# sharonct/CTPA-CLIP

Measured on AMD Instinct MI355X. Metric: CT-report pairs/sec (contrastive step), higher is better.
Workload: dtype bf16

## Files before the change

ctpa-clip_amd/csrc/attn.hip:

```cpp
#include "common.h"
#include "../../include/ctclip_hip.h"

namespace {

constexpr float LOG2E = 1.4426950408889634f;
constexpr float LN2 = 0.6931471805599453f;

struct AP {
  const u16* q; int64_t ldq;
  const u16* k; int64_t ldk;
  const u16* v; int64_t ldv;
  const u16* o; int64_t ldo;
  u16* out; int64_t ldout;
  u16* out16;
  const u16* dout; int64_t lddo;
  u16* dq; int64_t lddq;
  u16* dk; int64_t lddk;
  u16* dv; int64_t lddv;
  float* lse;
  float* delta;
  const float* bias_u;
  float* dbias_u;
  float* dbias_ws;
  const int32_t* kmask;
// ... 655 lines not shown
        pk.y = pack2(dq[d][2], dq[d][3]);
        *(uint2*)(p.dq + qrow * p.lddq + h * D + d * 16 + 4 * g) = pk;
      }
    }
  }
  if (BIAS && p.dbias_u) {
    __syncthreads();
    const int hh = blockIdx.x % p.H;
    for (int i = tid; i < p.nbins; i += NT) {
      const float v = bins[i];
      if (v != 0.f) atomicAdd(&p.dbias_u[(int64_t)hh * p.nbins + i], v);
    }
  }
}

template <int D, bool BIAS, int W = (BIAS ? 12 : NW), bool RUN = false>
__global__ __launch_bounds__(W * 64) void attn_bwd_dkv_kernel(AP p) {
  extern __shared__ __attribute__((aligned(16))) char smem[];
  constexpr int KK = D / 32, DB = D / 16, RS = Img<D>::RS, NTH = W * 64;
  const int L = p.L, Lp = (L + 31) & ~31;
  const int tid = threadIdx.x, lane = tid & 63, w = tid >> 6;
  const int wpp = W / p.pp;
  const int pair_local = w / wpp, wi = w - pair_local * wpp;
  const int pair_bytes = 2 * Lp * RS + 2 * Lp * 4;
  for (int pl = 0; pl < p.pp; ++pl) {
    const int pair = blockIdx.x * p.pp + pl;
    if (pair >= p.nseq * p.H) break;
    const int s = pair / p.H, h = pair - s * p.H;
    char* base = smem + pl * pair_bytes;
    stage2<D, SU>(base, p.q, p.ldq, base + Lp * RS, p.dout, p.lddo, p, s, h, Lp, tid, NTH);
    float* ls = (float*)(base + 2 * Lp * RS);
    float* dls = ls + Lp;
    for (int i = tid; i < Lp; i += NTH) {
      const bool v = i < L;
      const int64_t r = v ? seq_row(p, s, i) : 0;
      ls[i] = v ? p.lse[(int64_t)h * p.M + r] * LOG2E : INFINITY;
      dls[i] = v ? p.delta[(int64_t)h * p.M + r] : 0.f;
    }
  }
  float* ub = nullptr;
  int* kb = nullptr;
  float* madd = nullptr;
  load_tables<BIAS, NTH>(p, smem + p.pp * pair_bytes, Lp, tid, blockIdx.x % p.H, ub, kb, madd);
  __syncthreads();
  const int pair = blockIdx.x * p.pp + pair_local;
  if (pair >= p.nseq * p.H) return;
  const int s = pair / p.H, h = pair - s * p.H;
  const char* Qimg = smem + pair_local * pair_bytes;
  const char* Dimg = Qimg + Lp * RS;
  const float* ls = (const float*)(Qimg + 2 * Lp * RS);
  const float* dls = ls + Lp;
  const int g = lane >> 4, li = lane & 15;
  const int nkb = (L + 15) >> 4;
  const float sc2 = p.scale * LOG2E;
  for (int kbk = wi; kbk < nkb; kbk += wpp) {
    const int key = kbk * 16 + li;
    const bool kin = key < L;
    const float kadd = madd[pair_local * Lp + key];
    const int64_t krow = kin ? seq_row(p, s, key) : 0;
    bf16x8 kf[KK], vf[KK];
#pragma unroll
    for (int kk = 0; kk < KK; ++kk) {
      kf[kk] = kin ? gload8(p.k + krow * p.ldk + h * D + kk * 32 + 8 * g) : zero8();
      vf[kk] = kin ? gload8(p.v + krow * p.ldv + h * D + kk * 32 + 8 * g) : zero8();
    }
    const int ck = BIAS && kin ? kb[key] - boff(p) : 0;
    f32x4 dk[DB], dv[DB];
#pragma unroll
    for (int d = 0; d < DB; ++d) { dk[d] = f32x4{0.f, 0.f, 0.f, 0.f}; dv[d] = f32x4{0.f, 0.f, 0.f, 0.f}; }
    for (int qc = 0; qc < Lp; qc += 32) {
      f32x4 sa[2], da[2];
#pragma unroll
      for (int bi = 0; bi < 2; ++bi) {
        sa[bi] = f32x4{0.f, 0.f, 0.f, 0.f};
        da[bi] = f32x4{0.f, 0.f, 0.f, 0.f};
#pragma unroll
        for (int kk = 0; kk < KK; ++kk) {
          sa[bi] = __builtin_amdgcn_mfma_f32_16x16x32_bf16(rowfrag<D>(Qimg, qc + 16 * bi, kk, lane), kf[kk], sa[bi], 0, 0, 0);
          da[bi] = __builtin_amdgcn_mfma_f32_16x16x32_bf16(rowfrag<D>(Dimg, qc + 16 * bi, kk, lane), vf[kk], da[bi], 0, 0, 0);
        }
      }
#pragma unroll
      for (int bi = 0; bi < 2; ++bi) {
        const int q0 = qc + 16 * bi + 4 * g;
        const f32x4 lv = *(const f32x4*)(ls + q0);
        const f32x4 dlv = *(const f32x4*)(dls + q0);
        int4 qbv;
        const float* up = nullptr;
        if constexpr (RUN) up = ub + (kb[q0] - ck);
        else if (BIAS) qbv = *(const int4*)(kb + q0);
#pragma unroll
        for (int r = 0; r < 4; ++r) {
          float x;
          if constexpr (RUN) x = sa[bi][r] * sc2 + up[r];
          else x = sa[bi][r] * sc2 + kadd;
          if (BIAS && !RUN) x += ub[qbv[r] - ck];
          const float pr = fexp2(x - lv[r]);
          float keep = 1.f;
          if constexpr (!BIAS) {
            if (p.drop_p > 0.f) keep = drop_keep(p, s, h, q0 + r, key);
          }
          const float ds = pr * (da[bi][r] * keep - dlv[r]);
          sa[bi][r] = pr * keep;
          da[bi][r] = ds * p.scale;
        }
      }
      const bf16x8 pa = pack_perm(sa[0], sa[1]);
      const bf16x8 dsa = pack_perm(da[0], da[1]);
#pragma unroll
      for (int d = 0; d < DB; ++d) {
        dv[d] = __builtin_amdgcn_mfma_f32_16x16x32_bf16(pa, trfrag<D>(Dimg, qc, d * 16, lane), dv[d], 0, 0, 0);
        dk[d] = __builtin_amdgcn_mfma_f32_16x16x32_bf16(dsa, trfrag<D>(Qimg, qc, d * 16, lane), dk[d], 0, 0, 0);
      }
    }
#pragma unroll
    for (int r = 0; r < 4; ++r) {
      const int kr = kbk * 16 + 4 * g + r;
      if (kr >= L) continue;
      const int64_t row = seq_row(p, s, kr);
#pragma unroll
      for (int d = 0; d < DB; ++d) {
        p.dk[row * p.lddk + h * D + d * 16 + li] = f2bf(dk[d][r]);
        p.dv[row * p.lddv + h * D + d * 16 + li] = f2bf(dv[d][r]);
      }
    }
  }
}

template <int MAXCH, bool RUN = false>
__global__ __launch_bounds__(NT) void attn_bwd_dq_bias_kernel(AP p, int nfc) {
  extern __shared__ __attribute__((aligned(16))) char smem[];
  constexpr int D = 32, RS = Img<D>::RS, DB = 2;
  const int L = p.L, Lp = (L + 31) & ~31, nc = Lp / 32, nc0 = (nc + 1) / 2;
  const int tid = threadIdx.x, lane = tid & 63, w = tid >> 6;
  const int h = blockIdx.x, qg = blockIdx.y, fc = blockIdx.z;
  const int qsub = w & 3, khalf = w >> 2;
  const int c_begin = khalf ? nc0 : 0, c_end = khalf ? nc : nc0;
  char* Kimg = smem;
  char* Vimg = smem + Lp * RS;
  float* ub = (float*)(smem + 2 * Lp * RS);
  const int nb4 = (p.nbins + 3) & ~3;
  float* bins = ub + nb4;
  int* kb = (int*)(bins + nb4);
  float* madd = (float*)(kb + Lp);
  float* xch = madd + Lp;
  for (int i = tid; i < p.nbins; i += NT) { ub[i] = p.bias_u[(int64_t)h * p.nbins + i] * LOG2E; bins[i] = 0.f; }
  for (int i = tid; i < Lp; i += NT) {
    kb[i] = i < L ? kb_of(p, i) : 0;
    madd[i] = i < L ? 0.f : -INFINITY;
  }
  const int g = lane >> 4, li = lane & 15;
  const int q = qg * 64 + qsub * 16 + li;
  const bool qv = q < L;
  const float sc2 = p.scale * LOG2E;
  f32x4 acc[MAXCH][2];
#pragma unroll
  for (int c = 0; c < MAXCH; ++c) { acc[c][0] = f32x4{0.f, 0.f, 0.f, 0.f}; acc[c][1] = f32x4{0.f, 0.f, 0.f, 0.f}; }
  const int f0 = (int)((int64_t)p.nseq * fc / nfc), f1 = (int)((int64_t)p.nseq * (fc + 1) / nfc);
  __syncthreads();
  const int cq = kb[min(q, L - 1)] + boff(p);
  for (int s = f0; s < f1; ++s) {
    __syncthreads();
    stage2<D, SUB>(Kimg, p.k, p.ldk, Vimg, p.v, p.ldv, p, s, h, Lp, tid, NT);
    const int64_t qrow = qv ? seq_row(p, s, q) : 0;
    bf16x8 qf, df;
    float dl = 0.f;
    if (qv) {
      qf = gload8(p.q + qrow * p.ldq + h * D + 8 * g);
      df = gload8(p.dout + qrow * p.lddo + h * D + 8 * g);
      const bf16x8 of = gload8(p.o + qrow * p.ldo + h * D + 8 * g);
#pragma unroll
      for (int j = 0; j < 8; ++j) dl += (float)df[j] * (float)of[j];
    } else {
      qf = zero8();
      df = zero8();
    }
    dl += __shfl_xor(dl, 16, 64);
    dl += __shfl_xor(dl, 32, 64);
    const float lse2 = qv ? p.lse[(int64_t)h * p.M + qrow] * LOG2E : INFINITY;
    if (qv && g == 0 && khalf == 0) p.delta[(int64_t)h * p.M + qrow] = dl;
    __syncthreads();
    f32x4 dq[DB];
#pragma unroll
    for (int d = 0; d < DB; ++d) dq[d] = f32x4{0.f, 0.f, 0.f, 0.f};
#pragma unroll
    for (int ci = 0; ci < MAXCH; ++ci) {
      const int c = c_begin + ci;
      if (c < c_end) {
        const int kc = c * 32;
        f32x4 sa[2], da[2];
#pragma unroll
        for (int bi = 0; bi < 2; ++bi) {
          sa[bi] = __builtin_amdgcn_mfma_f32_16x16x32_bf16(rowfrag<D>(Kimg, kc + 16 * bi, 0, lane), qf,
                                                           f32x4{0.f, 0.f, 0.f, 0.f}, 0, 0, 0);
          da[bi] = __builtin_amdgcn_mfma_f32_16x16x32_bf16(rowfrag<D>(Vimg, kc + 16 * bi, 0, lane), df,
                                                           f32x4{0.f, 0.f, 0.f, 0.f}, 0, 0, 0);
        }
#pragma unroll
        for (int bi = 0; bi < 2; ++bi) {
          const int k0 = kc + 16 * bi + 4 * g;
          int4 kbv;
          f32x4 ma;
          const float* up = nullptr;
          if constexpr (RUN) {
            up = ub + (cq - kb[k0] - 3);
          } else {
            kbv = *(const int4*)(kb + k0);
            ma = *(const f32x4*)(madd + k0);
          }
#pragma unroll
          for (int r = 0; r < 4; ++r) {
            const float x = RUN ? sa[bi][r] * sc2 + up[3 - r] : sa[bi][r] * sc2 + ma[r] + ub[cq - kbv[r]];
            const float ds = fexp2(x - lse2) * (da[bi][r] - dl);
            acc[ci][bi][r] += ds;
            sa[bi][r] = ds * p.scale;
          }
        }
        const bf16x8 dsb = pack_perm(sa[0], sa[1]);
#pragma unroll
        for (int d = 0; d < DB; ++d)
          dq[d] = __builtin_amdgcn_mfma_f32_16x16x32_bf16(trfrag<D>(Kimg, kc, d * 16, lane), dsb, dq[d], 0, 0, 0);
      }
    }
    if (khalf == 1) {
#pragma unroll
      for (int d = 0; d < DB; ++d)
#pragma unroll
        for (int r = 0; r < 4; ++r) xch[(qsub * 64 + lane) * 8 + d * 4 + r] = dq[d][r];
    }
    __syncthreads();
    if (khalf == 0 && qv) {
#pragma unroll
      for (int d = 0; d < DB; ++d) {
        f32x4 v = dq[d];
#pragma unroll
        for (int r = 0; r < 4; ++r) v[r] += xch[(qsub * 64 + lane) * 8 + d * 4 + r];
        uint2 pk;
        pk.x = pack2(v[0], v[1]);
        pk.y = pack2(v[2], v[3]);
        *(uint2*)(p.dq + qrow * p.lddq + h * D + d * 16 + 4 * g) = pk;
      }
    }
  }
  {
    float* S = (float*)smem;
    const int LH = nc0 * 32;
    const int Wg = p.Wg, Hg = p.Hg, W2 = 2 * Wg - 1;
    for (int part = 0; part < 8; ++part) {
      const int ph = part >> 2, pq = part & 3;
      __syncthreads();
      if (khalf == ph && qsub == pq) {
#pragma unroll
        for (int ci = 0; ci < MAXCH; ++ci) {
          const int c = c_begin + ci;
          if (c < c_end) {
#pragma unroll
            for (int bi = 0; bi < 2; ++bi)
#pragma unroll
              for (int r = 0; r < 4; ++r) S[li * LH + (c - c_begin) * 32 + 16 * bi + 4 * g + r] = acc[ci][bi][r];
          }
        }
      }
      __syncthreads();
      const int k0 = ph * LH, k1 = min(L, k0 + LH);
      const int q0 = qg * 64 + pq * 16;
      for (int b = tid; b < p.nbins; b += NT) {
        const int dh = b / W2 - (Hg - 1), dw = b % W2 - (Wg - 1);
        float sum = 0.f;
        for (int j = 0; j < 16 && q0 + j < L; ++j) {
          const int qi = q0 + j, kh = qi / Wg - dh, kw = qi % Wg - dw;
          if (kh >= 0 && kh < Hg && kw >= 0 && kw < Wg) {
            const int key = kh * Wg + kw;
            if (key >= k0 && key < k1) sum += S[j * LH + key - k0];
          }
        }
        bins[b] += sum;
      }
    }
  }
  __syncthreads();
  for (int i = tid; i < p.nbins; i += NT) {
    const float v = bins[i];
    if (p.dbias_ws) p.dbias_ws[((int64_t)(qg * nfc + fc) * p.H + h) * p.nbins + i] = v;
    else if (v != 0.f) atomicAdd(&p.dbias_u[(int64_t)h * p.nbins + i], v);
  }
}

constexpr int DQD_W = 8, DQD_NT = DQD_W * 64, DQD_KP = 2;
#ifndef CTCLIP_ATTN_CFOLD
#define CTCLIP_ATTN_CFOLD 1
#endif
#ifndef CTCLIP_ATTN_CFOLD_DQ
#define CTCLIP_ATTN_CFOLD_DQ 0
#endif
#ifndef CTCLIP_ATTN_DQ_KBFAST
#define CTCLIP_ATTN_DQ_KBFAST 0
#endif
#ifndef CTCLIP_ATTN_DIAG_BIN
#define CTCLIP_ATTN_DIAG_BIN 1
#endif
#ifndef CTCLIP_ATTN_DQ_CINIT
#define CTCLIP_ATTN_DQ_CINIT 1
#endif
template <int LF, int KP = DQD_KP>
__global__ __launch_bounds__(4 * KP * 64) void attn_bwd_dq_bias_dma_kernel(AP p, int nfc) {
  extern __shared__ __attribute__((aligned(16))) char smem[];
  constexpr int D = 32, DB = 2, L = LF, NC = L / 32, NCP = NC / KP, NW = 4 * KP, NTH = NW * 64;
  constexpr int IMG = L * 64, BUF = 2 * IMG, NG = BUF / 1024 / NW;
  static_assert(L % 64 == 0 && NC % KP == 0 && (BUF / 1024) % NW == 0 && (IMG / 1024) % NG == 0 &&
                (KP - 1) * 4 * 64 * 8 * 4 <= BUF, "full-shape specialisation");
  const int tid = threadIdx.x, lane = tid & 63, w = tid >> 6;
  const int h = blockIdx.x, qg = blockIdx.y, fc = blockIdx.z;
  const int qsub = w & 3, kpart = w >> 2;
  const int c_begin = kpart * NCP;
  float* ub = (float*)(smem + 2 * BUF);
  const int nb4 = (p.nbins + 3) & ~3;
  int* kb = (int*)(ub + nb4);
#if CTCLIP_ATTN_DQ_CINIT
  {
    const float isc = 1.f / p.scale;
    for (int i = tid; i < p.nbins; i += NTH) ub[i] = p.bias_u[(int64_t)h * p.nbins + p.nbins - 1 - i] * isc;
  }
#else
  for (int i = tid; i < p.nbins; i += NTH) ub[i] = p.bias_u[(int64_t)h * p.nbins + i] * LOG2E;
#endif
  for (int i = tid; i < L; i += NTH) kb[i] = kb_of(p, i);
  const int g = lane >> 4, li = lane & 15;
  const int q = qg * 64 + qsub * 16 + li;
  const float sc2 = p.scale * LOG2E;
  f32x4 acc[NCP][2];
#pragma unroll
  for (int c = 0; c < NCP; ++c) { acc[c][0] = f32x4{0.f, 0.f, 0.f, 0.f}; acc[c][1] = f32x4{0.f, 0.f, 0.f, 0.f}; }
  const int f0 = (int)((int64_t)p.nseq * fc / nfc), f1 = (int)((int64_t)p.nseq * (fc + 1) / nfc);
  auto stage_frame = [&](int s, int b) {
    const int64_t fb = (int64_t)s * p.s_outer;
#pragma unroll
    for (int j = 0; j < NG; ++j) {
      const int pos = (w * NG + j) * 1024 + lane * 16;
      const bool isv = pos >= IMG;
      const int pi = isv ? pos - IMG : pos, row = pi >> 6, ch = ((pi >> 4) & 3) ^ kv_swz(row);
      const u16* src = isv ? p.v + (fb + row) * p.ldv : p.k + (fb + row) * p.ldk;
      glds16_asm(src + h * D + ch * 8, smem + b * BUF + (w * NG + j) * 1024);
    }
  };
  bf16x8 qf = zero8(), df = zero8(), of = zero8();
  float lse2 = 0.f;
  auto load_q = [&](int s) {
    const int64_t qrow = (int64_t)s * p.s_outer + q;
    qf = gload8(p.q + qrow * p.ldq + h * D + 8 * g);
    df = gload8(p.dout + qrow * p.lddo + h * D + 8 * g);
    of = gload8(p.o + qrow * p.ldo + h * D + 8 * g);
    lse2 = p.lse[(int64_t)h * p.M + qrow];
  };
  if (f0 < f1) {
    load_q(f0);
    stage_frame(f0, 0);
  }
  asm volatile("s_waitcnt lgkmcnt(0)" ::: "memory");
  __builtin_amdgcn_s_barrier();
  __builtin_amdgcn_sched_barrier(0);
  const int cq = kb[q] + boff(p);
  [[maybe_unused]] const int cqr = p.nbins - 1 - cq;
  [[maybe_unused]] const KbFast kbf = kb_fast_init(p);
  for (int s = f0; s < f1; ++s) {
    const int b = (s - f0) & 1;
    const char* Kimg = smem + b * BUF;
    const char* Vimg = Kimg + IMG;
    asm volatile("s_waitcnt vmcnt(0)" ::: "memory");
    __builtin_amdgcn_s_barrier();
    __builtin_amdgcn_sched_barrier(0);
    bf16x8 qc = qf, dc = df;
    float l2 = lse2 * LOG2E;
    float dl = 0.f;
#pragma unroll
    for (int j = 0; j < 8; ++j) dl += (float)df[j] * (float)of[j];
    dl += __shfl_xor(dl, 16, 64);
    dl += __shfl_xor(dl, 32, 64);
    {
      typedef unsigned int v4u __attribute__((ext_vector_type(4)));
      v4u qv = __builtin_bit_cast(v4u, qc), dv = __builtin_bit_cast(v4u, dc);
      asm volatile("" : "+v"(qv), "+v"(dv), "+v"(l2), "+v"(dl));
      qc = __builtin_bit_cast(bf16x8, qv);
      dc = __builtin_bit_cast(bf16x8, dv);
    }
    const int64_t qrow = (int64_t)s * p.s_outer + q;
    if (g == 0 && kpart == 0) p.delta[(int64_t)h * p.M + qrow] = dl;
#if CTCLIP_ATTN_CFOLD_DQ
    const float cl = -lse2 / p.scale;
    const f32x4 cS = f32x4{cl, cl, cl, cl}, cD = f32x4{-dl, -dl, -dl, -dl};
#else
    const f32x4 cS = f32x4{0.f, 0.f, 0.f, 0.f}, cD = cS;
#endif
    __builtin_amdgcn_sched_barrier(0);
    if (s + 1 < f1) {
      load_q(s + 1);
      stage_frame(s + 1, b ^ 1);
    }
    __builtin_amdgcn_sched_barrier(0);
    f32x4 dq[DB];
#pragma unroll
    for (int d = 0; d < DB; ++d) dq[d] = f32x4{0.f, 0.f, 0.f, 0.f};
#pragma unroll
    for (int ci = 0; ci < NCP; ++ci) {
      const int kc = (c_begin + ci) * 32;
      f32x4 sa[2], da[2];
#if CTCLIP_ATTN_DQ_CINIT
      (void)cS;
      const float nl2 = -l2;
#pragma unroll
      for (int bi = 0; bi < 2; ++bi) {
        const float* up = ub + (kb[kc + 16 * bi + 4 * g] + cqr);
        sa[bi] = __builtin_amdgcn_mfma_f32_16x16x32_bf16(rowfrag_sw(Kimg, kc + 16 * bi, lane), qc,
                                                         f32x4{up[0], up[1], up[2], up[3]}, 0, 0, 0);
        da[bi] = __builtin_amdgcn_mfma_f32_16x16x32_bf16(rowfrag_sw(Vimg, kc + 16 * bi, lane), dc, cD, 0, 0, 0);
      }
#pragma unroll
      for (int bi = 0; bi < 2; ++bi)
#pragma unroll
        for (int r = 0; r < 4; ++r) {
#if CTCLIP_ATTN_CFOLD_DQ
          const float ds = fexp2(fmaf(sa[bi][r], sc2, nl2)) * da[bi][r];
#else
          const float ds = fexp2(fmaf(sa[bi][r], sc2, nl2)) * (da[bi][r] - dl);
#endif
          acc[ci][bi][r] += ds;
          sa[bi][r] = ds;
        }
#else
#pragma unroll
      for (int bi = 0; bi < 2; ++bi) {
        sa[bi] = __builtin_amdgcn_mfma_f32_16x16x32_bf16(rowfrag_sw(Kimg, kc + 16 * bi, lane), qc, cS, 0, 0, 0);
        da[bi] = __builtin_amdgcn_mfma_f32_16x16x32_bf16(rowfrag_sw(Vimg, kc + 16 * bi, lane), dc, cD, 0, 0, 0);
      }
#pragma unroll
      for (int bi = 0; bi < 2; ++bi) {
        int k0 = kc + 16 * bi + 4 * g;
#if CTCLIP_ATTN_DQ_KBFAST
        asm volatile("" : "+v"(k0));
        const float* up = ub + (cq - kb_fast(kbf, k0) - 3);
#else
        const float* up = ub + (cq - kb[k0] - 3);
#endif
#pragma unroll
        for (int r = 0; r < 4; ++r) {
          const float x = sa[bi][r] * sc2 + up[3 - r];
#if CTCLIP_ATTN_CFOLD_DQ
          const float ds = fexp2(x) * da[bi][r];
#else
          const float ds = fexp2(x - l2) * (da[bi][r] - dl);
#endif
          acc[ci][bi][r] += ds;
          sa[bi][r] = ds;
        }
      }
#endif
      const bf16x8 dsb = pack_perm(sa[0], sa[1]);
#pragma unroll
      for (int d = 0; d < DB; ++d)
        dq[d] = __builtin_amdgcn_mfma_f32_16x16x32_bf16(trfrag_sw(Kimg, kc, d * 16, lane), dsb, dq[d], 0, 0, 0);
    }
#pragma unroll
    for (int d = 0; d < DB; ++d) dq[d] *= p.scale;
    float* xch = (float*)(smem + b * BUF);
    asm volatile("s_waitcnt lgkmcnt(0)" ::: "memory");
    __builtin_amdgcn_s_barrier();
    __builtin_amdgcn_sched_barrier(0);
    if (kpart > 0) {
#pragma unroll
      for (int d = 0; d < DB; ++d)
#pragma unroll
        for (int r = 0; r < 4; ++r) xch[(((kpart - 1) * 4 + qsub) * 64 + lane) * 8 + d * 4 + r] = dq[d][r];
    }
    asm volatile("s_waitcnt lgkmcnt(0)" ::: "memory");
    __builtin_amdgcn_s_barrier();
    __builtin_amdgcn_sched_barrier(0);
    if (kpart == 0) {
#pragma unroll
      for (int d = 0; d < DB; ++d) {
        f32x4 v = dq[d];
#pragma unroll
        for (int pp = 0; pp < KP - 1; ++pp)
#pragma unroll
          for (int r = 0; r < 4; ++r) v[r] += xch[((pp * 4 + qsub) * 64 + lane) * 8 + d * 4 + r];
        uint2 pk;
        pk.x = pack2(v[0], v[1]);
        pk.y = pack2(v[2], v[3]);
        *(uint2*)(p.dq + qrow * p.lddq + h * D + d * 16 + 4 * g) = pk;
      }
    }
  }
  asm volatile("s_waitcnt vmcnt(0) lgkmcnt(0)" ::: "memory");
  __syncthreads();
#if CTCLIP_ATTN_DIAG_BIN
  {
    constexpr int LP = L + 3;
    static_assert(64 * LP * 4 <= 2 * BUF + 4 * (2209 + 3) + 4 * L, "dS block fits the buffers and tables");
    float* S = (float*)smem;
    const int ql = qsub * 16 + li;
#pragma unroll
    for (int ci = 0; ci < NCP; ++ci)
#pragma unroll
      for (int bi = 0; bi < 2; ++bi)
#pragma unroll
        for (int r = 0; r < 4; ++r) S[ql * LP + (c_begin + ci) * 32 + 16 * bi + 4 * g + r] = acc[ci][bi][r];
    __syncthreads();
    const int Wg = p.Wg, Hg = p.Hg, W2 = 2 * Wg - 1, q0 = qg * 64;
    const int r_lo = q0 / Wg, r_hi = (q0 + 63) / Wg;
    for (int b = tid; b < p.nbins; b += NTH) {
      const int dh = b / W2 - (Hg - 1), dw = b % W2 - (Wg - 1);
      float sum = 0.f;
      for (int r = r_lo; r <= r_hi; ++r) {
        const int kh = r - dh;
        if (kh < 0 || kh >= Hg) continue;
        const int lo = max(max(q0 - r * Wg, 0), dw), hi = min(min(q0 + 63 - r * Wg, Wg - 1), Wg - 1 + dw);
        const float* sp = S + (r * Wg - q0) * LP + kh * Wg - dw;
        for (int qw = lo; qw <= hi; ++qw) sum += sp[qw * (LP + 1)];
      }
      if (p.dbias_ws) p.dbias_ws[((int64_t)(qg * nfc + fc) * p.H + h) * p.nbins + b] = sum;
      else if (sum != 0.f) atomicAdd(&p.dbias_u[(int64_t)h * p.nbins + b], sum);
    }
  }
#else
  float* bins = (float*)smem;
  for (int i = tid; i < p.nbins; i += NTH) bins[i] = 0.f;
  __syncthreads();
#ifndef CTCLIP_ATTN_NO_BIN
#pragma unroll
  for (int ci = 0; ci < NCP; ++ci)
#pragma unroll
    for (int bi = 0; bi < 2; ++bi)
#pragma unroll
      for (int r = 0; r < 4; ++r) {
        const int key = (c_begin + ci) * 32 + 16 * bi + 4 * g + r;
        atomicAdd(&bins[cq - kb[key]], acc[ci][bi][r]);
      }
#else
  if (acc[0][0][0] == 12345.f) bins[0] = 1.f;
#endif
  __syncthreads();
  for (int i = tid; i < p.nbins; i += NTH) {
    const float v = bins[i];
    if (v != 0.f) atomicAdd(&p.dbias_u[(int64_t)h * p.nbins + i], v);
  }
#endif
}

constexpr int DKP_W = 12, DKP_NT = DKP_W * 64;
template <int LF>
__global__ __launch_bounds__(DKP_NT) void attn_bwd_dkv_persist_kernel(AP p) {
  extern __shared__ __attribute__((aligned(16))) char smem[];
  constexpr int D = 32, DB = 2, RS = 64, W = DKP_W, NTH = DKP_NT, L = LF, CH = D / 8;
  constexpr int NLD = 2 * L * CH / NTH, RPU = NTH / CH, NKB = L / 16;
  static_assert((2 * L * CH) % NTH == 0 && L % 32 == 0 && L % 16 == 0 && (W * 64 / CH) % 16 == 0, "shape");
  const int tid = threadIdx.x, lane = tid & 63, wi = tid >> 6;
  const int h = blockIdx.x % p.H, wg = blockIdx.x / p.H, nwg = gridDim.x / p.H;
  char* Qimg = smem;
  char* Dimg = smem + L * RS;
  float* ls = (float*)(smem + 2 * L * RS);
  float* dls = ls + L;
  float* ub = dls + L;
  const int nb4 = (p.nbins + 3) & ~3;
  int* kb = (int*)(ub + nb4);
  for (int i = tid; i < p.nbins; i += NTH) ub[i] = p.bias_u[(int64_t)h * p.nbins + i] * LOG2E;
  for (int i = tid; i < L; i += NTH) kb[i] = kb_of(p, i);
  const int g = lane >> 4, li = lane & 15;
  const float sc2 = p.scale * LOG2E;
  const KbFast kbf = kb_fast_init(p);
  const int r0 = tid / CH, c0 = tid % CH;
  const int64_t offq = (int64_t)r0 * p.ldq + h * D + c0 * 8, offd = (int64_t)r0 * p.lddo + h * D + c0 * 8;
  u32x4 st[NLD];
  float lsv = 0.f, dlv = 0.f;
#define CT_DKV_LOAD(S_)                                                                          \
  do {                                                                                           \
    const int64_t fb_ = (int64_t)(S_) * p.s_outer;    \
    _Pragma("unroll") for (int u = 0; u < NLD; ++u) {                                            \
      const bool isq = u * RPU + (wi * 64) / CH < L;                                             \
      const u16* src_ = isq ? p.q + (fb_ + u * RPU) * p.ldq + offq : p.dout + (fb_ + u * RPU - L) * p.lddo + offd; \
      st[u] = *(const u32x4*)src_;                                                               \
    }                                                                                            \
    if (tid < L) {                                                                               \
      lsv = p.lse[(int64_t)h * p.M + fb_ + tid];                                                 \
      dlv = p.delta[(int64_t)h * p.M + fb_ + tid];                                               \
    }                                                                                            \
  } while (0)
  int s = wg;
  if (s < p.nseq) CT_DKV_LOAD(s);
  for (; s < p.nseq; s += nwg) {
    __syncthreads();
#pragma unroll
    for (int u = 0; u < NLD; ++u) {
      const bool isq = u * RPU + (wi * 64) / CH < L;
      char* dst = isq ? Qimg + (u * RPU) * RS : Dimg + (u * RPU - L) * RS;
      *(u32x4*)(dst + r0 * RS + ((c0 ^ kv_swz(u * RPU + r0)) << 4)) = st[u];
    }
    if (tid < L) {
      ls[tid] = lsv * LOG2E;
      dls[tid] = dlv;
    }
    __syncthreads();
    if (s + nwg < p.nseq) CT_DKV_LOAD(s + nwg);
    const int64_t fb = (int64_t)s * p.s_outer;
    bf16x8 kf = zero8(), vf = zero8();
    {
      const int64_t krow = fb + wi * 16 + li;
      kf = gload8(p.k + krow * p.ldk + h * D + 8 * g);
      vf = gload8(p.v + krow * p.ldv + h * D + 8 * g);
    }
    for (int kbk = wi; kbk < NKB; kbk += W) {
      const bf16x8 kc = kf, vc = vf;
      if (kbk + W < NKB) {
        const int64_t krow = fb + (kbk + W) * 16 + li;
        kf = gload8(p.k + krow * p.ldk + h * D + 8 * g);
        vf = gload8(p.v + krow * p.ldv + h * D + 8 * g);
      }
      const int key = kbk * 16 + li;
      const int ck = kb[key] - boff(p);
      f32x4 dk[DB], dv[DB];
#pragma unroll
      for (int d = 0; d < DB; ++d) { dk[d] = f32x4{0.f, 0.f, 0.f, 0.f}; dv[d] = f32x4{0.f, 0.f, 0.f, 0.f}; }
      for (int qc = 0; qc < L; qc += 32) {
        f32x4 sa[2], da[2];
#pragma unroll
        for (int bi = 0; bi < 2; ++bi) {
          sa[bi] = __builtin_amdgcn_mfma_f32_16x16x32_bf16(rowfrag_sw(Qimg, qc + 16 * bi, lane), kc,
                                                           f32x4{0.f, 0.f, 0.f, 0.f}, 0, 0, 0);
          da[bi] = __builtin_amdgcn_mfma_f32_16x16x32_bf16(rowfrag_sw(Dimg, qc + 16 * bi, lane), vc,
                                                           f32x4{0.f, 0.f, 0.f, 0.f}, 0, 0, 0);
        }
#pragma unroll
        for (int bi = 0; bi < 2; ++bi) {
          const int q0 = qc + 16 * bi + 4 * g;
          const f32x4 lv = *(const f32x4*)(ls + q0);
          const f32x4 dlq = *(const f32x4*)(dls + q0);
          const float* up = ub + (kb_fast(kbf, q0) - ck);
#pragma unroll
          for (int r = 0; r < 4; ++r) {
            const float x = sa[bi][r] * sc2 + up[r];
            const float pr = fexp2(x - lv[r]);
            const float ds = pr * (da[bi][r] - dlq[r]);
            sa[bi][r] = pr;
            da[bi][r] = ds;
          }
        }
        const bf16x8 pa = pack_perm(sa[0], sa[1]);
        const bf16x8 dsa = pack_perm(da[0], da[1]);
#pragma unroll
        for (int d = 0; d < DB; ++d) {
          dv[d] = __builtin_amdgcn_mfma_f32_16x16x32_bf16(pa, trfrag_sw(Dimg, qc, d * 16, lane), dv[d], 0, 0, 0);
          dk[d] = __builtin_amdgcn_mfma_f32_16x16x32_bf16(dsa, trfrag_sw(Qimg, qc, d * 16, lane), dk[d], 0, 0, 0);
        }
      }
#pragma unroll
      for (int d = 0; d < DB; ++d) dk[d] *= p.scale;
#pragma unroll
      for (int r = 0; r < 4; ++r) {
        const int64_t row = fb + kbk * 16 + 4 * g + r;
#pragma unroll
        for (int d = 0; d < DB; ++d) {
          p.dk[row * p.lddk + h * D + d * 16 + li] = f2bf(dk[d][r]);
          p.dv[row * p.lddv + h * D + d * 16 + li] = f2bf(dv[d][r]);
        }
      }
    }
  }
}
#undef CT_DKV_LOAD

constexpr int DKD_W = 12, DKD_NT = DKD_W * 64;
template <int LF>
__global__ __launch_bounds__(DKD_NT) void attn_bwd_dkv_dma_kernel(AP p) {
  extern __shared__ __attribute__((aligned(16))) char smem[];
  constexpr int D = 32, DB = 2, W = DKD_W, NTH = DKD_NT, L = LF, NKB = L / 16;
  constexpr int IMG = L * 64, BUF = 2 * IMG, NG = BUF / 1024 / W;
  static_assert(L % 32 == 0 && BUF % (1024 * W) == 0 && IMG % (1024 * NG) == 0 && NKB >= W, "full shape");
  const int tid = threadIdx.x, lane = tid & 63, wi = tid >> 6;
  const int h = blockIdx.x % p.H, wg = blockIdx.x / p.H, nwg = gridDim.x / p.H;
  float* ls = (float*)(smem + 2 * BUF);
  float* dls = ls + L;
  float* ub = dls + L;
  const int nb4 = (p.nbins + 3) & ~3;
  int* kb = (int*)(ub + nb4);
  for (int i = tid; i < p.nbins; i += NTH) ub[i] = p.bias_u[(int64_t)h * p.nbins + i] * LOG2E;
  for (int i = tid; i < L; i += NTH) kb[i] = kb_of(p, i);
  const int g = lane >> 4, li = lane & 15;
  const float sc2 = p.scale * LOG2E;
  const KbFast kbf = kb_fast_init(p);
  auto stage_frame = [&](int s, int b) {
    const int64_t fb = (int64_t)s * p.s_outer;
#pragma unroll
    for (int j = 0; j < NG; ++j) {
      const int pos = (wi * NG + j) * 1024 + lane * 16;
      const bool isd = pos >= IMG;
      const int pi = isd ? pos - IMG : pos, row = pi >> 6, ch = ((pi >> 4) & 3) ^ kv_swz(row);
      const u16* src = isd ? p.dout + (fb + row) * p.lddo : p.q + (fb + row) * p.ldq;
      glds16_asm(src + h * D + ch * 8, smem + b * BUF + (wi * NG + j) * 1024);
    }
  };
  float lsv = 0.f, dlv = 0.f;
  bf16x8 kf = zero8(), vf = zero8();
  auto load_kv = [&](int s, int kbk) {
    const int64_t krow = (int64_t)s * p.s_outer + kbk * 16 + li;
    kf = gload8(p.k + krow * p.ldk + h * D + 8 * g);
    vf = gload8(p.v + krow * p.ldv + h * D + 8 * g);
  };
  int s = wg;
  if (s < p.nseq) {
    stage_frame(s, 0);
    if (tid < L) {
      lsv = p.lse[(int64_t)h * p.M + (int64_t)s * p.s_outer + tid];
      dlv = p.delta[(int64_t)h * p.M + (int64_t)s * p.s_outer + tid];
    }
    load_kv(s, wi);
  }
  for (int it = 0; s < p.nseq; s += nwg, ++it) {
    const int b = it & 1;
    asm volatile("s_waitcnt vmcnt(0)" ::: "memory");
    __syncthreads();
    if (tid < L) {
#if CTCLIP_ATTN_CFOLD
      ls[tid] = -lsv / p.scale;
      dls[tid] = -dlv;
#else
      ls[tid] = lsv * LOG2E;
      dls[tid] = dlv;
#endif
    }
    __syncthreads();
    const int sn = s + nwg;
    if (sn < p.nseq) {
      stage_frame(sn, b ^ 1);
      if (tid < L) {
        lsv = p.lse[(int64_t)h * p.M + (int64_t)sn * p.s_outer + tid];
        dlv = p.delta[(int64_t)h * p.M + (int64_t)sn * p.s_outer + tid];
      }
    }
    const char* Qimg = smem + b * BUF;
    const char* Dimg = Qimg + IMG;
    const int64_t fb = (int64_t)s * p.s_outer;
    for (int kbk = wi; kbk < NKB; kbk += W) {
      const bf16x8 kc = kf, vc = vf;
      if (kbk + W < NKB) load_kv(s, kbk + W);
      else if (sn < p.nseq) load_kv(sn, wi);
      const int key = kbk * 16 + li;
      const int ck = kb[key] - boff(p);
      f32x4 dk[DB], dv[DB];
#pragma unroll
      for (int d = 0; d < DB; ++d) { dk[d] = f32x4{0.f, 0.f, 0.f, 0.f}; dv[d] = f32x4{0.f, 0.f, 0.f, 0.f}; }
      for (int qc = 0; qc < L; qc += 32) {
        f32x4 sa[2], da[2];
#pragma unroll
        for (int bi = 0; bi < 2; ++bi) {
#if CTCLIP_ATTN_CFOLD
          const int q0 = qc + 16 * bi + 4 * g;
          const f32x4 cS = *(const f32x4*)(ls + q0), cD = *(const f32x4*)(dls + q0);
#else
          const f32x4 cS = f32x4{0.f, 0.f, 0.f, 0.f}, cD = cS;
#endif
          sa[bi] = __builtin_amdgcn_mfma_f32_16x16x32_bf16(rowfrag_sw(Qimg, qc + 16 * bi, lane), kc, cS, 0, 0, 0);
          da[bi] = __builtin_amdgcn_mfma_f32_16x16x32_bf16(rowfrag_sw(Dimg, qc + 16 * bi, lane), vc, cD, 0, 0, 0);
        }
#pragma unroll
        for (int bi = 0; bi < 2; ++bi) {
          const int q0 = qc + 16 * bi + 4 * g;
#if !CTCLIP_ATTN_CFOLD
          const f32x4 lv = *(const f32x4*)(ls + q0);
          const f32x4 dlq = *(const f32x4*)(dls + q0);
#endif
          const float* up = ub + (kb_fast(kbf, q0) - ck);
#pragma unroll
          for (int r = 0; r < 4; ++r) {
            const float x = sa[bi][r] * sc2 + up[r];
#if CTCLIP_ATTN_CFOLD
            const float pr = fexp2(x);
            const float ds = pr * da[bi][r];
#else
            const float pr = fexp2(x - lv[r]);
            const float ds = pr * (da[bi][r] - dlq[r]);
#endif
            sa[bi][r] = pr;
            da[bi][r] = ds;
          }
        }
        const bf16x8 pa = pack_perm(sa[0], sa[1]);
        const bf16x8 dsa = pack_perm(da[0], da[1]);
#pragma unroll
        for (int d = 0; d < DB; ++d) {
          dv[d] = __builtin_amdgcn_mfma_f32_16x16x32_bf16(pa, trfrag_sw(Dimg, qc, d * 16, lane), dv[d], 0, 0, 0);
          dk[d] = __builtin_amdgcn_mfma_f32_16x16x32_bf16(dsa, trfrag_sw(Qimg, qc, d * 16, lane), dk[d], 0, 0, 0);
        }
      }
#pragma unroll
      for (int d = 0; d < DB; ++d) dk[d] *= p.scale;
#pragma unroll
// ... 598 lines not shown
```

Measured before the change: 210.5.

## Defer dQ cross-wave reduction to next frame and simplify DMA addressing

The cross-wave dQ exchange used to need two barriers per frame: one to write partials and one to read them. Now partials are written into the buffer just consumed, and the reduction and store happen at the start of the next frame, after the existing top-of-loop barrier. This removes one barrier per iteration, at the cost of a static constraint on exchange placement and an extra epilogue finish. Separately, the K/V staging address math is hoisted: the wave-uniform source, stride and row are computed once, leaving a per-lane offset plus a row stride per chunk. This cuts per-frame integer VALU work.

```diff
diff --git a/ctpa-clip_amd/csrc/attn.hip b/ctpa-clip_amd/csrc/attn.hip
--- a/ctpa-clip_amd/csrc/attn.hip
+++ b/ctpa-clip_amd/csrc/attn.hip
@@ -981,6 +981,12 @@
 #ifndef CTCLIP_ATTN_DQ_CINIT
 #define CTCLIP_ATTN_DQ_CINIT 1
 #endif
+#ifndef CTCLIP_ATTN_DQ_XCH_DEFER
+#define CTCLIP_ATTN_DQ_XCH_DEFER 1
+#endif
+#ifndef CTCLIP_ATTN_DQ_LEAN_ADDR
+#define CTCLIP_ATTN_DQ_LEAN_ADDR 1
+#endif
 template <int LF, int KP = DQD_KP>
 __global__ __launch_bounds__(4 * KP * 64) void attn_bwd_dq_bias_dma_kernel(AP p, int nfc) {
   extern __shared__ __attribute__((aligned(16))) char smem[];
@@ -988,6 +994,9 @@
   constexpr int IMG = L * 64, BUF = 2 * IMG, NG = BUF / 1024 / NW;
   static_assert(L % 64 == 0 && NC % KP == 0 && (BUF / 1024) % NW == 0 && (IMG / 1024) % NG == 0 &&
                 (KP - 1) * 4 * 64 * 8 * 4 <= BUF, "full-shape specialisation");
+#if CTCLIP_ATTN_DQ_XCH_DEFER
+  static_assert((KP - 1) * 64 * 8 * 4 <= NG * 1024, "exchange strip inside its reader's DMA region");
+#endif
   const int tid = threadIdx.x, lane = tid & 63, w = tid >> 6;
   const int h = blockIdx.x, qg = blockIdx.y, fc = blockIdx.z;
   const int qsub = w & 3, kpart = w >> 2;
@@ -1011,6 +1020,22 @@
 #pragma unroll
   for (int c = 0; c < NCP; ++c) { acc[c][0] = f32x4{0.f, 0.f, 0.f, 0.f}; acc[c][1] = f32x4{0.f, 0.f, 0.f, 0.f}; }
   const int f0 = (int)((int64_t)p.nseq * fc / nfc), f1 = (int)((int64_t)p.nseq * (fc + 1) / nfc);
+#if CTCLIP_ATTN_DQ_LEAN_ADDR
+  const int wu = __builtin_amdgcn_readfirstlane(w);
+  const bool dma_v = wu * NG * 1024 >= IMG;
+  const u16* const dma_src = dma_v ? p.v : p.k;
+  const int64_t dma_ld = dma_v ? p.ldv : p.ldk;
+  const int dma_row0 = (wu * NG * 1024 - (dma_v ? IMG : 0)) >> 6;
+  const int dma_lane = (lane >> 2) * (int)dma_ld + h * D + ((lane & 3) ^ kv_swz(lane >> 2)) * 8;
+  auto stage_frame = [&](int s, int b) {
+    int lo = dma_lane;
+    asm volatile("" : "+v"(lo));
+    const u16* src = dma_src + ((int64_t)s * p.s_outer + dma_row0) * dma_ld + lo;
+#pragma unroll
+    for (int j = 0; j < NG; ++j)
+      glds16_asm(src + j * 16 * dma_ld, smem + b * BUF + (wu * NG + j) * 1024);
+  };
+#else
   auto stage_frame = [&](int s, int b) {
     const int64_t fb = (int64_t)s * p.s_outer;
 #pragma unroll
@@ -1022,6 +1047,7 @@
       glds16_asm(src + h * D + ch * 8, smem + b * BUF + (w * NG + j) * 1024);
     }
   };
+#endif
   bf16x8 qf = zero8(), df = zero8(), of = zero8();
   float lse2 = 0.f;
   auto load_q = [&](int s) {
@@ -1041,11 +1067,39 @@
   const int cq = kb[q] + boff(p);
   [[maybe_unused]] const int cqr = p.nbins - 1 - cq;
   [[maybe_unused]] const KbFast kbf = kb_fast_init(p);
+#if CTCLIP_ATTN_DQ_XCH_DEFER
+  f32x4 dqh[DB];
+#pragma unroll
+  for (int d = 0; d < DB; ++d) dqh[d] = f32x4{0.f, 0.f, 0.f, 0.f};
+  auto finish_dq = [&](int sp, int bp) {
+    if (kpart == 0) {
+      const float* xch = (const float*)(smem + bp * BUF + qsub * (NG * 1024));
+      const int64_t qrow = (int64_t)sp * p.s_outer + q;
+#pragma unroll
+      for (int d = 0; d < DB; ++d) {
+        f32x4 v = dqh[d];
+#pragma unroll
+        for (int pp = 0; pp < KP - 1; ++pp)
+#pragma unroll
+          for (int r = 0; r < 4; ++r) v[r] += xch[(pp * 64 + lane) * 8 + d * 4 + r];
+        uint2 pk;
+        pk.x = pack2(v[0], v[1]);
+        pk.y = pack2(v[2], v[3]);
+        *(uint2*)(p.dq + qrow * p.lddq + h * D + d * 16 + 4 * g) = pk;
+      }
+    }
+    asm volatile("s_waitcnt lgkmcnt(0)" ::: "memory");
+  };
+#endif
   for (int s = f0; s < f1; ++s) {
     const int b = (s - f0) & 1;
     const char* Kimg = smem + b * BUF;
     const char* Vimg = Kimg + IMG;
+#if CTCLIP_ATTN_DQ_XCH_DEFER
+    asm volatile("s_waitcnt vmcnt(0) lgkmcnt(0)" ::: "memory");
+#else
     asm volatile("s_waitcnt vmcnt(0)" ::: "memory");
+#endif
     __builtin_amdgcn_s_barrier();
     __builtin_amdgcn_sched_barrier(0);
     bf16x8 qc = qf, dc = df;
@@ -1071,6 +1125,10 @@
     const f32x4 cS = f32x4{0.f, 0.f, 0.f, 0.f}, cD = cS;
 #endif
     __builtin_amdgcn_sched_barrier(0);
+#if CTCLIP_ATTN_DQ_XCH_DEFER
+    if (s > f0) finish_dq(s - 1, b ^ 1);
+    __builtin_amdgcn_sched_barrier(0);
+#endif
     if (s + 1 < f1) {
       load_q(s + 1);
       stage_frame(s + 1, b ^ 1);
@@ -1140,6 +1198,25 @@
     }
 #pragma unroll
     for (int d = 0; d < DB; ++d) dq[d] *= p.scale;
+#if CTCLIP_ATTN_DQ_XCH_DEFER
+    asm volatile("s_waitcnt lgkmcnt(0)" ::: "memory");
+    __builtin_amdgcn_s_barrier();
+    __builtin_amdgcn_sched_barrier(0);
+    if (kpart > 0) {
+      float* xch = (float*)(smem + b * BUF + qsub * (NG * 1024));
+#pragma unroll
+      for (int d = 0; d < DB; ++d)
+#pragma unroll
+        for (int r = 0; r < 4; ++r) xch[((kpart - 1) * 64 + lane) * 8 + d * 4 + r] = dq[d][r];
+    } else {
+#pragma unroll
+      for (int d = 0; d < DB; ++d) dqh[d] = dq[d];
+    }
+  }
+  asm volatile("s_waitcnt vmcnt(0) lgkmcnt(0)" ::: "memory");
+  __syncthreads();
+  if (f0 < f1) finish_dq(f1 - 1, (f1 - 1 - f0) & 1);
+#else
     float* xch = (float*)(smem + b * BUF);
     asm volatile("s_waitcnt lgkmcnt(0)" ::: "memory");
     __builtin_amdgcn_s_barrier();
@@ -1168,6 +1245,7 @@
       }
     }
   }
+#endif
   asm volatile("s_waitcnt vmcnt(0) lgkmcnt(0)" ::: "memory");
   __syncthreads();
 #if CTCLIP_ATTN_DIAG_BIN
```

Result: no change. 211.4 (median of 6 runs) (+0.4%).
